# shenyunhang/APE

Hardware: AMD Instinct MI355X
Metric: images/sec @1024^2 APE-L_D fwd (higher is better)
Workload: dtype bf16

## Files before the change

ape_amd/csrc/select.hip:

```cpp
#include "common.h"
#include "../../include/ape_hip.h"

__device__ __forceinline__ bool iou_gt(const float4 a, const float4 b, float thr) {
  const float area_a = (a.z - a.x) * (a.w - a.y);
  const float area_b = (b.z - b.x) * (b.w - b.y);
  const float xx1 = fmaxf(a.x, b.x), yy1 = fmaxf(a.y, b.y);
  const float xx2 = fminf(a.z, b.z), yy2 = fminf(a.w, b.w);
  const float w = fmaxf(0.f, xx2 - xx1), h = fmaxf(0.f, yy2 - yy1);
  const float inter = w * h;
  return inter / (area_a + area_b - inter) > thr;
}

__global__ __launch_bounds__(64) void nms_mask_kernel(const float4* __restrict__ boxes, const int* __restrict__ groups, int n,
                                                      float thr, unsigned long long* __restrict__ mask, int nw) {
  __shared__ float4 cb[64];
  __shared__ int cg[64];
  const int rb = blockIdx.y, cbk = blockIdx.x, t = threadIdx.x;
  const int j0 = cbk * 64;
  if (j0 + t < n) {
    cb[t] = boxes[j0 + t];
    cg[t] = groups ? groups[j0 + t] : 0;
  }
  __syncthreads();
  const int i = rb * 64 + t;
  if (i >= n) return;
  const float4 bi = boxes[i];
  const int gi = groups ? groups[i] : 0;
  unsigned long long bits = 0ull;
  const int cnt = min(64, n - j0);
  for (int j = 0; j < cnt; ++j) {
    if (j0 + j != i && cg[j] == gi && iou_gt(bi, cb[j], thr)) bits |= (1ull << j);
  }
  mask[(size_t)i * nw + cbk] = bits;
}

__device__ __forceinline__ unsigned long long readlane64(unsigned long long v, int lane_uniform) {
  const unsigned lo = (unsigned)__builtin_amdgcn_readlane((int)(unsigned)(v & 0xffffffffull), lane_uniform);
  const unsigned hi = (unsigned)__builtin_amdgcn_readlane((int)(unsigned)(v >> 32), lane_uniform);
  return ((unsigned long long)hi << 32) | lo;
}

__device__ __forceinline__ unsigned long long uniform64(unsigned long long v) {
  const unsigned lo = (unsigned)__builtin_amdgcn_readfirstlane((int)(unsigned)(v & 0xffffffffull));
  const unsigned hi = (unsigned)__builtin_amdgcn_readfirstlane((int)(unsigned)(v >> 32));
  return ((unsigned long long)hi << 32) | lo;
}
__device__ __forceinline__ unsigned long long wave_or64(unsigned long long v) {
  unsigned lo = (unsigned)(v & 0xffffffffull), hi = (unsigned)(v >> 32);
#pragma unroll
  for (int o = 32; o > 0; o >>= 1) { lo |= (unsigned)__shfl_xor((int)lo, o, 64); hi |= (unsigned)__shfl_xor((int)hi, o, 64); }
  return ((unsigned long long)hi << 32) | lo;
}

template <bool USE_LDS>
__global__ __launch_bounds__(256) void nms_scan_segments_kernel(const unsigned long long* __restrict__ mask, int nw, int n,
                                                                const int* __restrict__ seg, const uint8_t* __restrict__ valid,
                                                                uint8_t* __restrict__ keep) {
  extern __shared__ __attribute__((aligned(16))) unsigned long long sub[];
  const int s0 = seg[blockIdx.x], s1 = seg[blockIdx.x + 1];
  if (s1 <= s0) return;
  const int w0 = s0 >> 6, w1 = (s1 - 1) >> 6;
  const int nws = w1 - w0 + 1;
  const int r_base = w0 * 64;
  if (USE_LDS) {
    const int nrows = (w1 + 1) * 64 - r_base;
    for (int e = threadIdx.x; e < nrows * nws; e += 256) {
      const int r = e / nws, w = e - r * nws;
      const int row = r_base + r;
      sub[e] = row < n ? mask[(size_t)row * nw + w0 + w] : 0ull;
    }
    __syncthreads();
  }
  if (threadIdx.x >= 64) return;
  const int lane = threadIdx.x;
  auto word = [&](int row, int c) -> unsigned long long {
    if (USE_LDS) return sub[(size_t)(row - r_base) * nws + (c - w0)];
    return mask[(size_t)(row < n ? row : n - 1) * nw + c];
  };
  unsigned long long kept0 = 0ull, kept1 = 0ull;
  for (int c = w0; c <= w1; ++c) {
    unsigned long long acc = 0ull;
    for (int cp = w0; cp < c; cp += 8) {
      unsigned long long t[8];
#pragma unroll
      for (int u = 0; u < 8; ++u) {
        const int cq = cp + u;
        const int cqc = cq < c ? cq : cp;
        const int rel = cqc - w0;
        const unsigned long long km = readlane64(rel >= 64 ? kept1 : kept0, rel & 63);
        const bool take = cq < c && ((km >> lane) & 1ull);
        const unsigned long long v = word(cqc * 64 + lane, c);
        t[u] = take ? v : 0ull;
      }
#pragma unroll
      for (int u = 0; u < 8; ++u) acc |= t[u];
    }
    const unsigned long long remc = uniform64(wave_or64(acc));
    const int i = c * 64 + lane;
    const bool in_seg = i >= s0 && i < s1;
    const bool ok = in_seg && (valid == nullptr || valid[i] != 0);
    const unsigned long long row_c = ok ? word(i, c) : 0ull;
    unsigned long long alive = __builtin_amdgcn_ballot_w64(ok) & ~remc;
    unsigned long long kept = 0ull;
    while (alive != 0ull) {
      const int j = __builtin_ctzll(alive);
      kept |= 1ull << j;
      alive &= ~(1ull << j);
      alive &= ~readlane64(row_c, j);
    }
    if (in_seg) keep[i] = (uint8_t)((kept >> lane) & 1ull);
    const int rel = c - w0;
    if (lane == (rel & 63)) { if (rel >= 64) kept1 = kept; else kept0 = kept; }
  }
}

__global__ __launch_bounds__(256) void nms_scan_classes_kernel(const unsigned long long* __restrict__ mask, int nw, int n,
                                                               const int* __restrict__ order, const uint8_t* __restrict__ valid,
                                                               uint8_t* __restrict__ keep, int num_classes) {
  extern __shared__ __attribute__((aligned(16))) unsigned long long smask[];
  const int tid = threadIdx.x, lane = tid & 63, wave = tid >> 6;
  for (int i = tid; i < n * nw; i += 256) smask[i] = mask[i];
  __syncthreads();
  const int c = blockIdx.x * 4 + wave;
  if (c >= num_classes) return;
  const int* ord = order + (size_t)c * n;
  unsigned long long rem = 0ull;
  for (int base = 0; base < n; base += 64) {
    const int p = base + lane;
    const int qv = p < n ? ord[p] : 0;
    const int okv = (p < n) && (valid == nullptr || valid[(size_t)c * n + p] != 0);
    int keptv = 0;
    const int cnt = min(64, n - base);
    for (int u = 0; u < cnt; ++u) {
      const int qi = __builtin_amdgcn_readlane(qv, u);
      const int ok = __builtin_amdgcn_readlane(okv, u);
      const unsigned long long row = lane < nw ? smask[(size_t)qi * nw + lane] : 0ull;
      const unsigned long long r = readlane64(rem, qi >> 6);
      const bool kept = ok && !((r >> (qi & 63)) & 1ull);
      if (kept) rem |= row;
      if (lane == u) keptv = kept ? 1 : 0;
    }
    if (p < n) keep[(size_t)c * n + p] = (uint8_t)keptv;
  }
}

extern "C" int ape_hip_nms_mask_words(int n) { return ceil_div(n, 64); }

extern "C" int ape_hip_nms_mask(const float* boxes, const int* groups, int n, float iou_thr, uint64_t* mask, void* stream) {
  APE_CHECK_ARG(boxes && mask && n > 0 && ((uintptr_t)boxes) % 16 == 0, "ape_hip_nms_mask: bad args");
  const int nw = ceil_div(n, 64);
  APE_LAUNCH(nms_mask_kernel, dim3(nw, nw), dim3(64), 0, (hipStream_t)stream, (const float4*)boxes, groups, n, iou_thr,
                     (unsigned long long*)mask, nw);
  APE_CHECK_LAUNCH("ape_hip_nms_mask");
  return 0;
}

extern "C" int ape_hip_nms_scan_segments(const uint64_t* mask, int n, const int* seg_offsets, int num_segments, int max_segment,
                                         const uint8_t* valid, uint8_t* keep, void* stream) {
  APE_CHECK_ARG(mask && seg_offsets && keep && n > 0 && num_segments > 0, "ape_hip_nms_scan_segments: bad args");
  APE_CHECK_ARG(max_segment <= 126 * 64, "ape_hip_nms_scan_segments: segment longer than %d candidates", 126 * 64);
  const size_t sub_rows = (size_t)(ceil_div(max_segment, 64) + 1) * 64, sub_words = (size_t)ceil_div(max_segment, 64) + 1;
  const size_t lds = sub_rows * sub_words * 8;
  if (lds <= 160 * 1024) {
    static ApeOncePerDevice attr_done;
    if (attr_done.first()) {
      (void)hipFuncSetAttribute((const void*)nms_scan_segments_kernel<true>, hipFuncAttributeMaxDynamicSharedMemorySize, 160 * 1024);
    }
    APE_LAUNCH(nms_scan_segments_kernel<true>, dim3(num_segments), dim3(256), lds, (hipStream_t)stream,
                       (const unsigned long long*)mask, ceil_div(n, 64), n, seg_offsets, valid, keep);
  } else {
    APE_LAUNCH(nms_scan_segments_kernel<false>, dim3(num_segments), dim3(256), 0, (hipStream_t)stream,
                       (const unsigned long long*)mask, ceil_div(n, 64), n, seg_offsets, valid, keep);
  }
  APE_CHECK_LAUNCH("ape_hip_nms_scan_segments");
  return 0;
}

extern "C" int ape_hip_nms_scan_classes(const uint64_t* mask, int n, const int* order, int num_classes, const uint8_t* valid,
                                        uint8_t* keep, void* stream) {
  const int nw = ceil_div(n, 64);
  const size_t lds = (size_t)n * nw * 8;
  APE_CHECK_ARG(mask && order && keep && n > 0 && num_classes > 0 && lds <= 160 * 1024,
                "ape_hip_nms_scan_classes: bad args (the n x n/64 bit matrix must fit the 160 KiB LDS: n <= 1280)");
  static ApeOncePerDevice attr_done;
  if (attr_done.first()) {
    (void)hipFuncSetAttribute((const void*)nms_scan_classes_kernel, hipFuncAttributeMaxDynamicSharedMemorySize, 160 * 1024);
  }
  APE_LAUNCH(nms_scan_classes_kernel, dim3(ceil_div(num_classes, 4)), dim3(256), lds, (hipStream_t)stream,
                     (const unsigned long long*)mask, nw, n, order, valid, keep, num_classes);
  APE_CHECK_LAUNCH("ape_hip_nms_scan_classes");
  return 0;
}
```

ape_amd/csrc/topk.hip:

```cpp
#include "common.h"
#include "../../include/ape_hip.h"

typedef unsigned long long u64;
#define TK_THREADS 1024

__device__ __forceinline__ uint32_t ordkey(float x) {
  const uint32_t u = __float_as_uint(x);
  return u ^ ((u >> 31) ? 0xffffffffu : 0x80000000u);
}
__device__ __forceinline__ float ordkey_inv(uint32_t k) {
  return __uint_as_float(k ^ ((k >> 31) ? 0x80000000u : 0xffffffffu));
}
__device__ __forceinline__ float sigmoid_f(float x) { return 1.f / (1.f + expf(-x)); }

struct TkLevels {
  int start[8];
  int n[8];
  int L;
};
__device__ __forceinline__ int level_of(const TkLevels& lv, int idx) {
  int l = 0;
#pragma unroll
  for (int i = 1; i < 8; ++i) l += (i < lv.L && idx >= lv.start[i]) ? 1 : 0;
  return l;
}

template <int N>
__device__ __forceinline__ void bitonic_desc(u64* s) {
  for (int k = 2; k <= N; k <<= 1) {
    for (int j = k >> 1; j > 0; j >>= 1) {
      for (int i = threadIdx.x; i < N; i += TK_THREADS) {
        const int p = i ^ j;
        if (p > i) {
          const u64 a = s[i], b = s[p];
          const bool first_larger = (i & k) == 0;
          if (first_larger ? (a < b) : (a > b)) { s[i] = b; s[p] = a; }
        }
      }
      __syncthreads();
    }
  }
}

template <typename KeyFn>
__device__ __forceinline__ void radix_select(KeyFn key, int n, int k, uint32_t* hist, uint32_t* sh, uint32_t& thr, uint32_t& rem) {
  uint32_t prefix = 0, r = (uint32_t)k;
  for (int shift = 24; shift >= 0; shift -= 8) {
    for (int b = threadIdx.x; b < 256; b += TK_THREADS) hist[b] = 0;
    __syncthreads();
    const uint32_t himask = shift == 24 ? 0u : (0xffffffffu << (shift + 8));
    for (int i0 = 0; i0 < n; i0 += TK_THREADS) {
      const int i = i0 + threadIdx.x;
      const uint32_t kk = i < n ? key(i) : 0u;
      bool live = i < n && (kk & himask) == prefix;
      const uint32_t bin = (kk >> shift) & 255u;
      u64 todo = __ballot(live);
      while (todo) {
        const int leader = __ffsll((long long)todo) - 1;
        const uint32_t lb = (uint32_t)__builtin_amdgcn_readlane((int)bin, leader);
        const u64 same = __ballot(live && bin == lb);
        if ((int)(threadIdx.x & 63) == leader) atomicAdd(&hist[lb], (uint32_t)__popcll(same));
        todo &= ~same;
        if (live && bin == lb) live = false;
      }
    }
    __syncthreads();
    if (threadIdx.x == 0) {
      uint32_t cum = 0;
      int b = 255;
      for (; b > 0; --b) {
        if (cum + hist[b] >= r) break;
        cum += hist[b];
      }
      sh[0] = prefix | ((uint32_t)b << shift);
      sh[1] = r - cum;
    }
    __syncthreads();
    prefix = sh[0];
    r = sh[1];
    __syncthreads();
  }
  thr = prefix;
  rem = r;
}

template <typename KeyFn, typename CompFn>
__device__ __forceinline__ void block_topk(KeyFn key, CompFn composite, int n, int k, u64* comp, uint32_t* hist, uint32_t* sh, uint32_t* wcnt) {
  comp[threadIdx.x] = 0ull;
  __syncthreads();
  if (n <= k) {
    for (int i = threadIdx.x; i < n; i += TK_THREADS) comp[i] = composite(i);
    __syncthreads();
  } else {
    uint32_t thr, rem;
    radix_select(key, n, k, hist, sh, thr, rem);
    const uint32_t ngt = (uint32_t)k - rem;
    const int lane = threadIdx.x & 63, wave = threadIdx.x >> 6;
    uint32_t base_gt = 0, base_eq = 0;
    for (int i0 = 0; i0 < n; i0 += TK_THREADS) {
      const int i = i0 + threadIdx.x;
      const uint32_t kk = i < n ? key(i) : 0u;
      const bool gt = i < n && kk > thr, eq = i < n && kk == thr;
      const u64 bg = __ballot(gt), be = __ballot(eq);
      const u64 lt = (1ull << lane) - 1ull;
      if (lane == 0) { wcnt[wave] = (uint32_t)__popcll(bg); wcnt[16 + wave] = (uint32_t)__popcll(be); }
      __syncthreads();
      uint32_t wg = 0, we = 0, tg = 0, te = 0;
#pragma unroll
      for (int w = 0; w < 16; ++w) {
        const uint32_t cg = wcnt[w], ce = wcnt[16 + w];
        if (w < wave) { wg += cg; we += ce; }
        tg += cg; te += ce;
      }
      if (gt) comp[base_gt + wg + (uint32_t)__popcll(bg & lt)] = composite(i);
      if (eq) {
        const uint32_t rank = base_eq + we + (uint32_t)__popcll(be & lt);
        if (rank < rem) comp[ngt + rank] = composite(i);
      }
      base_gt += tg;
      base_eq += te;
      __syncthreads();
    }
  }
  bitonic_desc<1024>(comp);
}

template <int PER>
__device__ __forceinline__ void block_topk_regs(const uint32_t (&kk)[PER], int n, int k, uint32_t gbase, u64* comp, uint32_t* hist,
                                                uint32_t* sh, uint32_t* wcnt) {
  comp[threadIdx.x] = 0ull;
  __syncthreads();
  const int lane = threadIdx.x & 63, wave = threadIdx.x >> 6;
  if (n <= k) {
    if ((int)threadIdx.x < n) comp[threadIdx.x] = ((u64)kk[0] << 32) | (u64)(0xffffffffu - (gbase + threadIdx.x));
    __syncthreads();
  } else {
    uint32_t prefix = 0, r = (uint32_t)k;
    for (int shift = 24; shift >= 0; shift -= 8) {
      for (int b = threadIdx.x; b < 256; b += TK_THREADS) hist[b] = 0;
      __syncthreads();
      const uint32_t himask = shift == 24 ? 0u : (0xffffffffu << (shift + 8));
#pragma unroll
      for (int j = 0; j < PER; ++j) {
        const int e = j * TK_THREADS + threadIdx.x;
        bool live = e < n && (kk[j] & himask) == prefix;
        const uint32_t bin = (kk[j] >> shift) & 255u;
        u64 todo = __ballot(live);
        while (todo) {
          const int leader = __ffsll((long long)todo) - 1;
          const uint32_t lb = (uint32_t)__builtin_amdgcn_readlane((int)bin, leader);
          const u64 same = __ballot(live && bin == lb);
          if (lane == leader) atomicAdd(&hist[lb], (uint32_t)__popcll(same));
          todo &= ~same;
          if (live && bin == lb) live = false;
        }
      }
      __syncthreads();
      if (threadIdx.x == 0) {
        uint32_t cum = 0;
        int b = 255;
        for (; b > 0; --b) {
          if (cum + hist[b] >= r) break;
          cum += hist[b];
        }
        sh[0] = prefix | ((uint32_t)b << shift);
        sh[1] = r - cum;
      }
      __syncthreads();
      prefix = sh[0];
      r = sh[1];
      __syncthreads();
    }
    const uint32_t thr = prefix, rem = r, ngt = (uint32_t)k - rem;
    uint32_t base_gt = 0, base_eq = 0;
#pragma unroll
    for (int j = 0; j < PER; ++j) {
      const int e = j * TK_THREADS + threadIdx.x;
      const bool gt = e < n && kk[j] > thr, eq = e < n && kk[j] == thr;
      const u64 bg = __ballot(gt), be = __ballot(eq);
      const u64 lt = (1ull << lane) - 1ull;
      if (lane == 0) { wcnt[wave] = (uint32_t)__popcll(bg); wcnt[16 + wave] = (uint32_t)__popcll(be); }
      __syncthreads();
      uint32_t wg = 0, we = 0, tg = 0, te = 0;
#pragma unroll
      for (int w = 0; w < 16; ++w) {
        const uint32_t cg = wcnt[w], ce = wcnt[16 + w];
        if (w < wave) { wg += cg; we += ce; }
        tg += cg; te += ce;
      }
      const u64 c = ((u64)kk[j] << 32) | (u64)(0xffffffffu - (gbase + (uint32_t)e));
      if (gt) comp[base_gt + wg + (uint32_t)__popcll(bg & lt)] = c;
      if (eq) {
        const uint32_t rank = base_eq + we + (uint32_t)__popcll(be & lt);
        if (rank < rem) comp[ngt + rank] = c;
      }
      base_gt += tg;
      base_eq += te;
      __syncthreads();
    }
  }
  bitonic_desc<1024>(comp);
}

#define TK_STAGE2_MAX 12288
#define TK_MAX_JOBS 96
struct TkJobs {
  int njobs, nseg;
  int seg_first[8], seg_jobs[8], seg_k[8], seg_n[8], seg_mode[8];
  int start[TK_MAX_JOBS], n[TK_MAX_JOBS], seg[TK_MAX_JOBS];
};

__device__ __forceinline__ void stage2_gather(const u64* __restrict__ ws, int first_job, int njobs, int k, u64* lds) {
  const int m = njobs * k;
  for (int i = threadIdx.x; i < m; i += TK_THREADS) lds[i] = ws[(size_t)(first_job + i / k) * 1024 + (i % k)];
  __syncthreads();
}

__global__ __launch_bounds__(256) void enc_finalize_kernel(const float* __restrict__ cls2, const float* __restrict__ d,
                                                           const float* __restrict__ anchors, int T, float* __restrict__ enc_class,
                                                           float* __restrict__ enc_coord, float* __restrict__ xyxy) {
  const int t = blockIdx.x * 256 + threadIdx.x;
  if (t >= T) return;
  const float2 c = *reinterpret_cast<const float2*>(cls2 + 2 * (size_t)t);
  const bool pick = c.y > c.x;
  enc_class[t] = pick ? c.y : c.x;
  const float4 dd = *reinterpret_cast<const float4*>(d + 8 * (size_t)t + (pick ? 4 : 0));
  const float4 a = *reinterpret_cast<const float4*>(anchors + 4 * (size_t)t);
  const float4 u = make_float4(dd.x + a.x, dd.y + a.y, dd.z + a.z, dd.w + a.w);
  *reinterpret_cast<float4*>(enc_coord + 4 * (size_t)t) = u;
  const float cx = sigmoid_f(u.x), cy = sigmoid_f(u.y), w = sigmoid_f(u.z), h = sigmoid_f(u.w);
  float4 b = make_float4(cx - 0.5f * w, cy - 0.5f * h, cx + 0.5f * w, cy + 0.5f * h);
  b.x = fminf(fmaxf(b.x, 0.f), 1.f); b.y = fminf(fmaxf(b.y, 0.f), 1.f);
  b.z = fminf(fmaxf(b.z, 0.f), 1.f); b.w = fminf(fmaxf(b.w, 0.f), 1.f);
  *reinterpret_cast<float4*>(xyxy + 4 * (size_t)t) = b;
}

template <int PER>
__global__ __launch_bounds__(TK_THREADS) void topk_stage1_kernel(const float* __restrict__ x, TkJobs jobs, u64* __restrict__ ws) {
  __shared__ u64 comp[1024];
  __shared__ uint32_t hist[256], sh[2], wcnt[32];
  const int job = blockIdx.x, seg = jobs.seg[job], start = jobs.start[job], n = jobs.n[job];
  const bool sig = jobs.seg_mode[seg] != 0;
  uint32_t kk[PER];
#pragma unroll
  for (int j = 0; j < PER; ++j) {
    const int e = j * TK_THREADS + threadIdx.x;
    const float v = e < n ? x[start + e] : 0.f;
    kk[j] = e < n ? ordkey(sig ? sigmoid_f(v) : v + 0.f) : 0u;
  }
  block_topk_regs<PER>(kk, n, jobs.seg_k[seg], (uint32_t)start, comp, hist, sh, wcnt);
  ws[(size_t)job * 1024 + threadIdx.x] = comp[threadIdx.x];
}

__global__ __launch_bounds__(TK_THREADS) void proposal_topk2_kernel(const u64* __restrict__ ws, TkJobs jobs, TkLevels lv, int k, int k_alt,
                                                                    int32_t* __restrict__ cand, int32_t* __restrict__ alt) {
  extern __shared__ u64 lds[];
  __shared__ u64 comp[1024];
  __shared__ uint32_t hist[256], sh[2], wcnt[32];
  const int l = blockIdx.x;
  const int kk = jobs.seg_k[l], m = jobs.seg_jobs[l] * kk;
  stage2_gather(ws, jobs.seg_first[l], jobs.seg_jobs[l], kk, lds);
  auto key = [&](int i) { return (uint32_t)(lds[i] >> 32); };
  auto composite = [&](int i) { return lds[i]; };
  block_topk(key, composite, m, kk, comp, hist, sh, wcnt);
  if (l == lv.L) {
    for (int r = threadIdx.x; r < k_alt; r += TK_THREADS) alt[r] = (int32_t)(0xffffffffu - (uint32_t)(comp[r] & 0xffffffffull));
    return;
  }
  const int start = lv.start[l], n = lv.n[l];
  const int own = n < k ? n : k;
  for (int r = threadIdx.x; r < k; r += TK_THREADS) {
    int idx;
    if (r < own) {
      idx = (int)(0xffffffffu - (uint32_t)(comp[r] & 0xffffffffull));
    } else {
      const int e = r - n;
      idx = e >= start ? e + n : e;
    }
    cand[l * k + r] = idx;
  }
}

__device__ __forceinline__ void scan5(const uint32_t v[5], uint32_t out[5], uint32_t tot[5], u64* sa, uint32_t* sb) {
  const int lane = threadIdx.x & 63, wave = threadIdx.x >> 6;
  u64 a = (u64)v[0] | ((u64)v[1] << 16) | ((u64)v[2] << 32) | ((u64)v[3] << 48);
  uint32_t b = v[4];
  u64 ia = a;
  uint32_t ib = b;
#pragma unroll
  for (int o = 1; o < 64; o <<= 1) {
    const uint32_t lo = __shfl_up((uint32_t)(ia & 0xffffffffull), o, 64), hi = __shfl_up((uint32_t)(ia >> 32), o, 64);
    const uint32_t tb = __shfl_up(ib, o, 64);
    if (lane >= o) { ia += ((u64)hi << 32) | lo; ib += tb; }
  }
  __syncthreads();
  if (lane == 63) { sa[wave] = ia; sb[wave] = ib; }
  __syncthreads();
  u64 wa = 0, ta = 0;
  uint32_t wb = 0, tb2 = 0;
#pragma unroll
  for (int w = 0; w < 16; ++w) {
    if (w < wave) { wa += sa[w]; wb += sb[w]; }
    ta += sa[w]; tb2 += sb[w];
  }
  const u64 ea = wa + ia - a;
  out[0] = (uint32_t)(ea & 0xffff); out[1] = (uint32_t)((ea >> 16) & 0xffff); out[2] = (uint32_t)((ea >> 32) & 0xffff);
  out[3] = (uint32_t)((ea >> 48) & 0xffff); out[4] = wb + ib - b;
  tot[0] = (uint32_t)(ta & 0xffff); tot[1] = (uint32_t)((ta >> 16) & 0xffff); tot[2] = (uint32_t)((ta >> 32) & 0xffff);
  tot[3] = (uint32_t)((ta >> 48) & 0xffff); tot[4] = tb2;
}

#define PO_PAD 8192
#define PO_PER (PO_PAD / TK_THREADS)
__global__ __launch_bounds__(TK_THREADS) void proposal_order_kernel(const int32_t* __restrict__ cand, int n, const float* __restrict__ logit,
                                                                    const float* __restrict__ xyxy, TkLevels lv,
                                                                    float* __restrict__ boxes_b, int32_t* __restrict__ groups_b,
                                                                    int32_t* __restrict__ seg, int32_t* __restrict__ cand_a,
                                                                    int32_t* __restrict__ lv_a, int32_t* __restrict__ pos_b) {
  extern __shared__ u64 po_lds[];
  __shared__ u64 sa[16];
  __shared__ uint32_t sb[16];
  const int nchunks = (n + 1023) >> 10, npad = nchunks << 10;
  u64* work = po_lds;
  u64* srt = po_lds + npad;
  for (int p = threadIdx.x; p < npad; p += TK_THREADS)
    work[p] = p < n ? (((u64)ordkey(logit[cand[p]] + 0.f) << 32) | (u64)(0xffffffffu - (uint32_t)p)) : (u64)(npad - 1 - p);
  __syncthreads();
  for (int k = 2; k <= 1024; k <<= 1) {
    for (int j = k >> 1; j > 0; j >>= 1) {
      for (int i = threadIdx.x; i < npad; i += TK_THREADS) {
        const int q = i ^ j;
        if (q > i) {
          const u64 a = work[i], b = work[q];
          const bool first_larger = ((i & 1023) & k) == 0;
          if (first_larger ? (a < b) : (a > b)) { work[i] = b; work[q] = a; }
        }
      }
      __syncthreads();
    }
  }
  for (int i = threadIdx.x; i < npad; i += TK_THREADS) {
    const u64 v = work[i];
    const int c = i >> 10;
    int rank = i & 1023;
    for (int o = 0; o < nchunks; ++o) {
      if (o == c) continue;
      const u64* ch = work + (o << 10);
      int lo = 0, hi = 1024;
      while (lo < hi) {
        const int mid = (lo + hi) >> 1;
        if (ch[mid] > v) lo = mid + 1; else hi = mid;
      }
      rank += lo;
    }
    srt[rank] = v;
  }
  __syncthreads();
  int idx[PO_PER], lev[PO_PER];
  uint32_t cnt[5] = {0, 0, 0, 0, 0};
#pragma unroll
  for (int j = 0; j < PO_PER; ++j) {
    const int a = threadIdx.x * PO_PER + j;
    idx[j] = -1; lev[j] = 0;
    if (a < n) {
      const int p = (int)(0xffffffffu - (uint32_t)(srt[a] & 0xffffffffull));
      idx[j] = cand[p];
      lev[j] = level_of(lv, idx[j]);
      cnt[lev[j]] += 1;
    }
  }
  uint32_t ex[5], tot[5];
  scan5(cnt, ex, tot, sa, sb);
  uint32_t segs[6];
  segs[0] = 0;
#pragma unroll
  for (int l = 0; l < 5; ++l) segs[l + 1] = segs[l] + tot[l];
  if (threadIdx.x == 0)
    for (int l = 0; l <= lv.L; ++l) seg[l] = (int32_t)segs[l];
#pragma unroll
  for (int j = 0; j < PO_PER; ++j) {
    const int a = threadIdx.x * PO_PER + j;
    if (a < n) {
      const int l = lev[j];
      const int b = (int)(segs[l] + ex[l]);
      ex[l] += 1;
      cand_a[a] = idx[j]; lv_a[a] = l; pos_b[a] = b;
      groups_b[b] = l;
      *reinterpret_cast<float4*>(boxes_b + 4 * (size_t)b) = *reinterpret_cast<const float4*>(xyxy + 4 * (size_t)idx[j]);
    }
  }
}

__global__ __launch_bounds__(TK_THREADS) void proposal_quota_kernel(const int32_t* __restrict__ cand_a, const int32_t* __restrict__ lv_a,
                                                                    const int32_t* __restrict__ pos_b, const uint8_t* __restrict__ keep_b,
                                                                    int n, const int32_t* __restrict__ alt, int n_alt, TkLevels lv, int nq,
                                                                    long long* __restrict__ out) {
  __shared__ u64 sa[16];
  __shared__ uint32_t sb[16];
  int X[PO_PER], lev[PO_PER];
  bool valid[PO_PER];
  uint32_t c[5] = {0, 0, 0, 0, 0};
#pragma unroll
  for (int j = 0; j < PO_PER; ++j) {
    const int a = threadIdx.x * PO_PER + j;
    X[j] = 0; lev[j] = 0; valid[j] = false;
    if (a < n) {
      X[j] = cand_a[a]; lev[j] = lv_a[a];
      valid[j] = keep_b[pos_b[a]] != 0;
      c[0] += valid[j] ? 1u : 0u;
    }
  }
  uint32_t ex[5], tot[5];
  scan5(c, ex, tot, sa, sb);
  const bool use_alt = (int)tot[0] < nq;
  if (use_alt) {
#pragma unroll
    for (int j = 0; j < PO_PER; ++j) {
      const int a = threadIdx.x * PO_PER + j;
      valid[j] = a < n && a < n_alt;
      X[j] = valid[j] ? alt[a] : 0;
      lev[j] = level_of(lv, X[j]);
    }
  }
  for (int r = threadIdx.x; r < nq; r += TK_THREADS) out[r] = 0;
#pragma unroll
  for (int l = 0; l < 5; ++l) c[l] = 0;
#pragma unroll
  for (int j = 0; j < PO_PER; ++j)
    if (valid[j]) c[lev[j]] += 1;
  scan5(c, ex, tot, sa, sb);
  const uint32_t quota = (uint32_t)(nq / lv.L);
  bool sel[PO_PER];
  uint32_t c2[5] = {0, 0, 0, 0, 0};
#pragma unroll
  for (int j = 0; j < PO_PER; ++j) {
    sel[j] = false;
    if (valid[j]) {
      sel[j] = ex[lev[j]] < quota;
      ex[lev[j]] += 1;
      c2[sel[j] ? 0 : 1] += 1;
    }
  }
  scan5(c2, ex, tot, sa, sb);
  const uint32_t need = (uint32_t)nq - tot[0];
  uint32_t c3[5] = {0, 0, 0, 0, 0};
  uint32_t rest = ex[1];
#pragma unroll
  for (int j = 0; j < PO_PER; ++j) {
    if (valid[j] && !sel[j]) {
      if (rest < need) sel[j] = true;
      rest += 1;
    }
    c3[0] += sel[j] ? 1u : 0u;
  }
  scan5(c3, ex, tot, sa, sb);
  uint32_t slot = ex[0];
#pragma unroll
  for (int j = 0; j < PO_PER; ++j)
    if (sel[j]) {
      if (slot < (uint32_t)nq) out[slot] = (long long)X[j];
      slot += 1;
    }
}

__global__ __launch_bounds__(64) void det_boxes_kernel(const float* __restrict__ logits, int ldl, int K, const float* __restrict__ boxes,
                                                       const float* __restrict__ scale, float* __restrict__ xyxy,
                                                       uint8_t* __restrict__ finite) {
  const int q = blockIdx.x, lane = threadIdx.x;
  bool ok = true;
  for (int c = lane; c < K; c += 64) ok = ok && isfinite(sigmoid_f(logits[(size_t)q * ldl + c]));
  ok = __ballot(!ok) == 0ull;
  if (lane == 0) {
    const float4 b = *reinterpret_cast<const float4*>(boxes + 4 * (size_t)q);
    const float4 s = *reinterpret_cast<const float4*>(scale);
    float4 o = make_float4((b.x - 0.5f * b.z) * s.x, (b.y - 0.5f * b.w) * s.y, (b.x + 0.5f * b.z) * s.z, (b.y + 0.5f * b.w) * s.w);
    ok = ok && isfinite(o.x) && isfinite(o.y) && isfinite(o.z) && isfinite(o.w);
    o.x = fminf(fmaxf(o.x, 0.f), s.x); o.y = fminf(fmaxf(o.y, 0.f), s.y);
    o.z = fminf(fmaxf(o.z, 0.f), s.z); o.w = fminf(fmaxf(o.w, 0.f), s.w);
    if (!ok) o = make_float4(0.f, 0.f, 0.f, 0.f);
    *reinterpret_cast<float4*>(xyxy + 4 * (size_t)q) = o;
    finite[q] = ok ? 1 : 0;
  }
}

__global__ __launch_bounds__(TK_THREADS) void class_sort_kernel(const float* __restrict__ logits, int ldl, int Q, const uint8_t* __restrict__ finite,
                                                                float thresh, float* __restrict__ sorted, int32_t* __restrict__ order,
                                                                uint8_t* __restrict__ valid) {
  __shared__ u64 comp[1024];
  const int c = blockIdx.x, q = threadIdx.x;
  comp[q] = q < Q ? (((u64)ordkey(sigmoid_f(logits[(size_t)q * ldl + c])) << 32) | (u64)(0xffffffffu - (uint32_t)q)) : 0ull;
  __syncthreads();
  bitonic_desc<1024>(comp);
  if (q < Q) {
    const float s = ordkey_inv((uint32_t)(comp[q] >> 32));
    const int src = (int)(0xffffffffu - (uint32_t)(comp[q] & 0xffffffffull));
    sorted[(size_t)c * Q + q] = s;
    order[(size_t)c * Q + q] = src;
    valid[(size_t)c * Q + q] = (s > thresh && finite[src]) ? 1 : 0;
  }
}

template <int PER>
__global__ __launch_bounds__(TK_THREADS) void det_topk1_kernel(const float* __restrict__ sorted, const uint8_t* __restrict__ keep, int total,
                                                               int k, u64* __restrict__ ws) {
  __shared__ u64 comp[1024];
  __shared__ uint32_t hist[256], sh[2], wcnt[32];
  const int start = blockIdx.x * (PER * TK_THREADS);
  const int n = min(PER * TK_THREADS, total - start);
  uint32_t kk[PER];
#pragma unroll
  for (int j = 0; j < PER; ++j) {
    const int e = j * TK_THREADS + threadIdx.x;
    kk[j] = e < n ? ordkey(keep[start + e] ? sorted[start + e] : -1.f) : 0u;
  }
  block_topk_regs<PER>(kk, n, k, (uint32_t)start, comp, hist, sh, wcnt);
  ws[(size_t)blockIdx.x * 1024 + threadIdx.x] = comp[threadIdx.x];
}

__global__ __launch_bounds__(TK_THREADS) void topk_merge_kernel(const u64* __restrict__ in, int nlists, int group, int k, u64* __restrict__ out) {
  extern __shared__ u64 lds[];
  __shared__ u64 comp[1024];
  __shared__ uint32_t hist[256], sh[2], wcnt[32];
  const int first = blockIdx.x * group;
  const int cnt = min(group, nlists - first);
  stage2_gather(in, first, cnt, k, lds);
  auto key = [&](int i) { return (uint32_t)(lds[i] >> 32); };
  auto composite = [&](int i) { return lds[i]; };
  block_topk(key, composite, cnt * k, k, comp, hist, sh, wcnt);
  out[(size_t)blockIdx.x * 1024 + threadIdx.x] = comp[threadIdx.x];
}

__global__ __launch_bounds__(TK_THREADS) void det_topk2_kernel(const u64* __restrict__ ws, int nchunks, const int32_t* __restrict__ order,
                                                               const float* __restrict__ xyxy, int Q, int k, float* __restrict__ det_boxes,
                                                               float* __restrict__ det_scores, long long* __restrict__ det_classes,
                                                               long long* __restrict__ det_query) {
  extern __shared__ u64 lds[];
  __shared__ u64 comp[1024];
  __shared__ uint32_t hist[256], sh[2], wcnt[32];
  stage2_gather(ws, 0, nchunks, k, lds);
  auto key = [&](int i) { return (uint32_t)(lds[i] >> 32); };
  auto composite = [&](int i) { return lds[i]; };
  block_topk(key, composite, nchunks * k, k, comp, hist, sh, wcnt);
  for (int r = threadIdx.x; r < k; r += TK_THREADS) {
    const int flat = (int)(0xffffffffu - (uint32_t)(comp[r] & 0xffffffffull));
    const int qi = order[flat];
    det_scores[r] = ordkey_inv((uint32_t)(comp[r] >> 32));
    det_classes[r] = (long long)(flat / Q);
    det_query[r] = (long long)qi;
    *reinterpret_cast<float4*>(det_boxes + 4 * (size_t)r) = *reinterpret_cast<const float4*>(xyxy + 4 * (size_t)qi);
  }
}

static int fill_levels(TkLevels& lv, const int* level_start, const int* level_n, int L) {
  APE_CHECK_ARG(level_start && level_n && L >= 1 && L <= 5, "proposal selection: 1 <= levels <= 5");
  for (int i = 0; i < 8; ++i) { lv.start[i] = i < L ? level_start[i] : 0x7fffffff; lv.n[i] = i < L ? level_n[i] : 0; }
  lv.L = L;
  return 0;
}

extern "C" int ape_hip_enc_finalize(const float* cls2, const float* d, const float* anchors, int T, float* enc_class, float* enc_coord,
                                    float* xyxy, void* stream) {
  APE_CHECK_ARG(cls2 && d && anchors && enc_class && enc_coord && xyxy && T > 0, "ape_hip_enc_finalize: bad arguments");
  APE_LAUNCH(enc_finalize_kernel, dim3(ceil_div(T, 256)), dim3(256), 0, (hipStream_t)stream, cls2, d, anchors, T, enc_class,
                     enc_coord, xyxy);
  APE_CHECK_LAUNCH("enc_finalize_kernel");
  return 0;
}

static int topk_per(const int* seg_n, const int* seg_k, int nseg) {
  const int pers[3] = {8, 32, 64};
  for (int pi = 0; pi < 3; ++pi) {
    bool ok = true;
    int jobs = 0;
    for (int s = 0; s < nseg; ++s) {
      const int c = ceil_div(seg_n[s], pers[pi] * TK_THREADS);
      ok = ok && (long long)c * seg_k[s] <= TK_STAGE2_MAX;
      jobs += c;
    }
    if (ok && jobs <= TK_MAX_JOBS) return pers[pi];
  }
  return 0;
}

static void set_stage2_attr() {
  static ApeOncePerDevice done;
  if (done.first()) {
    (void)hipFuncSetAttribute((const void*)proposal_topk2_kernel, hipFuncAttributeMaxDynamicSharedMemorySize, 112 * 1024);
    (void)hipFuncSetAttribute((const void*)det_topk2_kernel, hipFuncAttributeMaxDynamicSharedMemorySize, 112 * 1024);
    (void)hipFuncSetAttribute((const void*)topk_merge_kernel, hipFuncAttributeMaxDynamicSharedMemorySize, 112 * 1024);
  }
}

extern "C" int ape_hip_topk_workspace_words(int n_total) {
  const int det = ceil_div(n_total > 0 ? n_total : 1, 8 * TK_THREADS);
  const int lists = det > TK_MAX_JOBS ? det : TK_MAX_JOBS;
  return 1024 * (lists + lists / 2 + 1);
}

extern "C" int ape_hip_proposal_topk(const float* logit, int T, const int* level_start, const int* level_n, int L, int k, int k_alt,
                                     uint64_t* workspace, int32_t* cand, int32_t* alt, void* stream) {
  TkLevels lv;
  if (fill_levels(lv, level_start, level_n, L)) return -1;
  APE_CHECK_ARG(logit && workspace && cand && alt && T > 0 && k >= 1 && k <= 1024 && k_alt >= 1 && k_alt <= 1024 && k <= T && k_alt <= T,
                "ape_hip_proposal_topk: 1 <= k, k_alt <= min(1024, T)");
  int seg_n[8], seg_k[8];
  for (int l = 0; l < L; ++l) { seg_n[l] = level_n[l]; seg_k[l] = k; }
  seg_n[L] = T; seg_k[L] = k_alt;
  const int per = topk_per(seg_n, seg_k, L + 1);
  APE_CHECK_ARG(per > 0, "ape_hip_proposal_topk: %d tokens do not fit the two-stage selection", T);
  TkJobs jobs;
  memset(&jobs, 0, sizeof(jobs));
  jobs.nseg = L + 1;
  const int chunk = per * TK_THREADS;
  for (int s = 0; s <= L; ++s) {
    const int base = s < L ? level_start[s] : 0;
    jobs.seg_first[s] = jobs.njobs; jobs.seg_k[s] = seg_k[s]; jobs.seg_n[s] = seg_n[s]; jobs.seg_mode[s] = s < L ? 1 : 0;
    for (int c0 = 0; c0 < seg_n[s]; c0 += chunk) {
      jobs.start[jobs.njobs] = base + c0; jobs.n[jobs.njobs] = seg_n[s] - c0 < chunk ? seg_n[s] - c0 : chunk; jobs.seg[jobs.njobs] = s;
      ++jobs.njobs;
    }
    jobs.seg_jobs[s] = jobs.njobs - jobs.seg_first[s];
  }
  hipStream_t st = (hipStream_t)stream;
  u64* ws = reinterpret_cast<u64*>(workspace);
  if (per == 8) APE_LAUNCH(topk_stage1_kernel<8>, dim3(jobs.njobs), dim3(TK_THREADS), 0, st, logit, jobs, ws);
  else if (per == 32) APE_LAUNCH(topk_stage1_kernel<32>, dim3(jobs.njobs), dim3(TK_THREADS), 0, st, logit, jobs, ws);
  else APE_LAUNCH(topk_stage1_kernel<64>, dim3(jobs.njobs), dim3(TK_THREADS), 0, st, logit, jobs, ws);
  set_stage2_attr();
  int mmax = 0;
  for (int s = 0; s <= L; ++s) mmax = mmax > jobs.seg_jobs[s] * jobs.seg_k[s] ? mmax : jobs.seg_jobs[s] * jobs.seg_k[s];
  APE_LAUNCH(proposal_topk2_kernel, dim3(L + 1), dim3(TK_THREADS), (size_t)mmax * sizeof(u64), st, ws, jobs, lv, k, k_alt, cand, alt);
  APE_CHECK_LAUNCH("proposal_topk");
  return 0;
}

extern "C" int ape_hip_proposal_order(const int32_t* cand, int n, const float* logit, const float* xyxy, const int* level_start,
                                      const int* level_n, int L, float* boxes_b, int32_t* groups_b, int32_t* seg, int32_t* cand_a,
                                      int32_t* lv_a, int32_t* pos_b, void* stream) {
  TkLevels lv;
  if (fill_levels(lv, level_start, level_n, L)) return -1;
  APE_CHECK_ARG(cand && logit && xyxy && boxes_b && groups_b && seg && cand_a && lv_a && pos_b && n > 0 && n <= PO_PAD,
                "ape_hip_proposal_order: 1 <= n <= 8192 candidates");
  static ApeOncePerDevice attr_done;
  if (attr_done.first()) {
    (void)hipFuncSetAttribute((const void*)proposal_order_kernel, hipFuncAttributeMaxDynamicSharedMemorySize, 2 * PO_PAD * sizeof(u64));
  }
  APE_LAUNCH(proposal_order_kernel, dim3(1), dim3(TK_THREADS), (size_t)2 * ((n + 1023) / 1024) * 1024 * sizeof(u64), (hipStream_t)stream, cand, n, logit, xyxy, lv,
                     boxes_b, groups_b, seg, cand_a, lv_a, pos_b);
  APE_CHECK_LAUNCH("proposal_order_kernel");
  return 0;
}

extern "C" int ape_hip_proposal_quota(const int32_t* cand_a, const int32_t* lv_a, const int32_t* pos_b, const uint8_t* keep_b, int n,
                                      const int32_t* alt, int n_alt, const int* level_start, const int* level_n, int L, int nq,
                                      int64_t* out, void* stream) {
  TkLevels lv;
  if (fill_levels(lv, level_start, level_n, L)) return -1;
  APE_CHECK_ARG(cand_a && lv_a && pos_b && keep_b && alt && out && n > 0 && n <= PO_PAD && n_alt >= 0 && nq > 0,
                "ape_hip_proposal_quota: bad arguments (n <= 8192)");
  APE_LAUNCH(proposal_quota_kernel, dim3(1), dim3(TK_THREADS), 0, (hipStream_t)stream, cand_a, lv_a, pos_b, keep_b, n, alt, n_alt,
                     lv, nq, (long long*)out);
  APE_CHECK_LAUNCH("proposal_quota_kernel");
  return 0;
}

extern "C" int ape_hip_det_sort(const float* logits, int ldl, int Q, int K, const float* boxes, const float* scale, float thresh,
                                float* xyxy, uint8_t* finite, float* sorted, int32_t* order, uint8_t* valid, void* stream) {
  APE_CHECK_ARG(logits && boxes && scale && xyxy && finite && sorted && order && valid && K > 0, "ape_hip_det_sort: bad arguments");
  APE_CHECK_ARG(Q > 0 && Q <= 1024, "ape_hip_det_sort: 1 <= queries <= 1024 (got %d)", Q);
  hipStream_t st = (hipStream_t)stream;
  APE_LAUNCH(det_boxes_kernel, dim3(Q), dim3(64), 0, st, logits, ldl, K, boxes, scale, xyxy, finite);
  APE_LAUNCH(class_sort_kernel, dim3(K), dim3(TK_THREADS), 0, st, logits, ldl, Q, finite, thresh, sorted, order, valid);
  APE_CHECK_LAUNCH("ape_hip_det_sort");
  return 0;
}

extern "C" int ape_hip_det_topk(const float* sorted, const uint8_t* keep, const int32_t* order, const float* xyxy, int K, int Q, int k,
                                uint64_t* workspace, float* det_boxes, float* det_scores, int64_t* det_classes, int64_t* det_query,
                                void* stream) {
  APE_CHECK_ARG(sorted && keep && order && xyxy && workspace && det_boxes && det_scores && det_classes && det_query, "ape_hip_det_topk: null pointer");
  APE_CHECK_ARG(K > 0 && Q > 0 && (long long)K * Q < 0x7fffffffLL && k >= 1 && k <= 1024 && k <= K * Q, "ape_hip_det_topk: 1 <= k <= min(1024, K*Q)");
  const int total = K * Q;
  int per = topk_per(&total, &k, 1);
  const bool merge = per == 0;
  if (merge) per = 64;
  int nchunks = ceil_div(total, per * TK_THREADS);
  hipStream_t st = (hipStream_t)stream;
  u64* ws = reinterpret_cast<u64*>(workspace);
  if (per == 8) APE_LAUNCH(det_topk1_kernel<8>, dim3(nchunks), dim3(TK_THREADS), 0, st, sorted, keep, total, k, ws);
  else if (per == 32) APE_LAUNCH(det_topk1_kernel<32>, dim3(nchunks), dim3(TK_THREADS), 0, st, sorted, keep, total, k, ws);
  else APE_LAUNCH(det_topk1_kernel<64>, dim3(nchunks), dim3(TK_THREADS), 0, st, sorted, keep, total, k, ws);
  set_stage2_attr();
  if (merge) {
    const int cap_lists = ape_hip_topk_workspace_words(total) / 1024;
    u64* a = ws;
    u64* b = ws + (size_t)1024 * (cap_lists - (cap_lists / 3));
    const int group = TK_STAGE2_MAX / k;
    while ((long long)nchunks * k > TK_STAGE2_MAX) {
      const int nout = ceil_div(nchunks, group);
      APE_LAUNCH(topk_merge_kernel, dim3(nout), dim3(TK_THREADS), (size_t)group * k * sizeof(u64), st, a, nchunks, group, k, b);
      u64* t = a; a = b; b = t;
      nchunks = nout;
    }
    ws = a;
  }
  APE_LAUNCH(det_topk2_kernel, dim3(1), dim3(TK_THREADS), (size_t)nchunks * k * sizeof(u64), st, ws, nchunks, order, xyxy, Q, k,
                     det_boxes, det_scores, (long long*)det_classes, (long long*)det_query);
  APE_CHECK_LAUNCH("det_topk");
  return 0;
}
```

Baseline: 117.9.

## Rework NMS scans and top-k selection with register sorts and staged LDS

The segment NMS scan now stages mask columns into LDS in column groups, double-buffered, so three waves prefetch the next group while one wave scans. This replaces the old fallback that read from global memory whenever the segment did not fit. The per-class NMS scan now skips suppressed candidates in bulk via ballots instead of walking every candidate serially, and gains a global-memory fallback. Top-k and class sorting replace LDS bitonic sorts with register and lane-shuffle bitonic networks, and the stage-2 selection no longer gathers into dynamic LDS. These post-processing kernels are a small share of the end-to-end forward pass, and the large rewrite carries correctness risk.

Result: no change. 118.6, median of 6 (+0.6%).

```diff
diff --git a/ape_amd/csrc/select.hip b/ape_amd/csrc/select.hip
--- a/ape_amd/csrc/select.hip
+++ b/ape_amd/csrc/select.hip
@@ -52,95 +52,131 @@
   return ((unsigned long long)hi << 32) | lo;
 }
 
-template <bool USE_LDS>
+__device__ __forceinline__ void nms_stage_columns(const unsigned long long* __restrict__ mask, int nw, int n, int r_base, int c_first, int ncols,
+                                                  int nrows, int rows_cap, unsigned long long* buf, int tid, int nthreads) {
+  const int total = nrows * ncols;
+  for (int e0 = tid; e0 < total; e0 += 8 * nthreads) {
+    unsigned long long v[8];
+#pragma unroll
+    for (int u = 0; u < 8; ++u) {
+      const int e = min(e0 + u * nthreads, total - 1);
+      const int r = e / ncols, w = e - r * ncols;
+      v[u] = mask[(size_t)min(r_base + r, n - 1) * nw + c_first + w];
+    }
+#pragma unroll
+    for (int u = 0; u < 8; ++u) {
+      const int e = e0 + u * nthreads;
+      const int r = e / ncols, w = e - r * ncols;
+      if (e < total) buf[(size_t)w * rows_cap + r] = r_base + r < n ? v[u] : 0ull;
+    }
+  }
+}
+
 __global__ __launch_bounds__(256) void nms_scan_segments_kernel(const unsigned long long* __restrict__ mask, int nw, int n,
                                                                 const int* __restrict__ seg, const uint8_t* __restrict__ valid,
-                                                                uint8_t* __restrict__ keep) {
+                                                                uint8_t* __restrict__ keep, int gcols, int rows_cap) {
   extern __shared__ __attribute__((aligned(16))) unsigned long long sub[];
   const int s0 = seg[blockIdx.x], s1 = seg[blockIdx.x + 1];
   if (s1 <= s0) return;
   const int w0 = s0 >> 6, w1 = (s1 - 1) >> 6;
-  const int nws = w1 - w0 + 1;
   const int r_base = w0 * 64;
-  if (USE_LDS) {
-    const int nrows = (w1 + 1) * 64 - r_base;
-    for (int e = threadIdx.x; e < nrows * nws; e += 256) {
-      const int r = e / nws, w = e - r * nws;
-      const int row = r_base + r;
-      sub[e] = row < n ? mask[(size_t)row * nw + w0 + w] : 0ull;
+  if ((w1 - w0 + 1) * 64 > rows_cap) return;
+  const int lane = threadIdx.x & 63, wave = threadIdx.x >> 6;
+  const int ngroups = (w1 - w0 + gcols) / gcols;
+  auto group_cols = [&](int g) { return min(gcols, w1 + 1 - (w0 + g * gcols)); };
+  auto group_rows = [&](int g) { return (g * gcols + group_cols(g)) * 64; };
+  nms_stage_columns(mask, nw, n, r_base, w0, group_cols(0), group_rows(0), rows_cap, sub, threadIdx.x, 256);
+  __syncthreads();
+  unsigned long long kept0 = 0ull, kept1 = 0ull;
+  for (int g = 0; g < ngroups; ++g) {
+    const unsigned long long* cur = sub + (size_t)(g & 1) * gcols * rows_cap;
+    const int c_lo = w0 + g * gcols, c_hi = c_lo + group_cols(g) - 1;
+    if (wave != 0) {
+      if (g + 1 < ngroups)
+        nms_stage_columns(mask, nw, n, r_base, c_lo + gcols, group_cols(g + 1), group_rows(g + 1), rows_cap,
+                          sub + (size_t)((g + 1) & 1) * gcols * rows_cap, threadIdx.x - 64, 192);
+    } else {
+      auto word = [&](int row, int c) -> unsigned long long {
+        return cur[(size_t)(c - c_lo) * rows_cap + (row - r_base)];
+      };
+      for (int c = c_lo; c <= c_hi; ++c) {
+        unsigned long long acc = 0ull;
+        for (int cp = w0; cp < c; cp += 8) {
+          unsigned long long t[8];
+#pragma unroll
+          for (int u = 0; u < 8; ++u) {
+            const int cq = cp + u;
+            const int cqc = cq < c ? cq : cp;
+            const int rel = cqc - w0;
+            const unsigned long long km = readlane64(rel >= 64 ? kept1 : kept0, rel & 63);
+            const bool take = cq < c && ((km >> lane) & 1ull);
+            const unsigned long long v = word(cqc * 64 + lane, c);
+            t[u] = take ? v : 0ull;
+          }
+#pragma unroll
+          for (int u = 0; u < 8; ++u) acc |= t[u];
+        }
+        const unsigned long long remc = uniform64(wave_or64(acc));
+        const int i = c * 64 + lane;
+        const bool in_seg = i >= s0 && i < s1;
+        const bool ok = in_seg && (valid == nullptr || valid[i] != 0);
+        const unsigned long long row_c = ok ? word(i, c) : 0ull;
+        unsigned long long alive = __builtin_amdgcn_ballot_w64(ok) & ~remc;
+        unsigned long long kept = 0ull;
+        while (alive != 0ull) {
+          const int j = __builtin_ctzll(alive);
+          kept |= 1ull << j;
+          alive &= ~(1ull << j);
+          alive &= ~readlane64(row_c, j);
+        }
+        if (in_seg) keep[i] = (uint8_t)((kept >> lane) & 1ull);
+        const int rel = c - w0;
+        if (lane == (rel & 63)) { if (rel >= 64) kept1 = kept; else kept0 = kept; }
+      }
     }
     __syncthreads();
   }
-  if (threadIdx.x >= 64) return;
-  const int lane = threadIdx.x;
-  auto word = [&](int row, int c) -> unsigned long long {
-    if (USE_LDS) return sub[(size_t)(row - r_base) * nws + (c - w0)];
-    return mask[(size_t)(row < n ? row : n - 1) * nw + c];
-  };
-  unsigned long long kept0 = 0ull, kept1 = 0ull;
-  for (int c = w0; c <= w1; ++c) {
-    unsigned long long acc = 0ull;
-    for (int cp = w0; cp < c; cp += 8) {
-      unsigned long long t[8];
-#pragma unroll
-      for (int u = 0; u < 8; ++u) {
-        const int cq = cp + u;
-        const int cqc = cq < c ? cq : cp;
-        const int rel = cqc - w0;
-        const unsigned long long km = readlane64(rel >= 64 ? kept1 : kept0, rel & 63);
-        const bool take = cq < c && ((km >> lane) & 1ull);
-        const unsigned long long v = word(cqc * 64 + lane, c);
-        t[u] = take ? v : 0ull;
-      }
-#pragma unroll
-      for (int u = 0; u < 8; ++u) acc |= t[u];
-    }
-    const unsigned long long remc = uniform64(wave_or64(acc));
-    const int i = c * 64 + lane;
-    const bool in_seg = i >= s0 && i < s1;
-    const bool ok = in_seg && (valid == nullptr || valid[i] != 0);
-    const unsigned long long row_c = ok ? word(i, c) : 0ull;
-    unsigned long long alive = __builtin_amdgcn_ballot_w64(ok) & ~remc;
+}
+
+template <bool IN_LDS>
+__global__ __launch_bounds__(256) void nms_scan_classes_kernel(const unsigned long long* __restrict__ mask, int nw, int n,
+                                                               const int* __restrict__ order, const uint8_t* __restrict__ valid,
+                                                               uint8_t* __restrict__ keep, int num_classes) {
+  extern __shared__ __attribute__((aligned(16))) unsigned long long lds_mask[];
+  const int tid = threadIdx.x, lane = tid & 63, wave = tid >> 6;
+  if (IN_LDS) {
+    for (int i = tid; i < n * nw; i += 256) lds_mask[i] = mask[i];
+    __syncthreads();
+  }
+  const unsigned long long* smask = IN_LDS ? lds_mask : mask;
+  const int c = blockIdx.x * 4 + wave;
+  if (c >= num_classes) return;
+  const int* ord = order + (size_t)c * n;
+  const uint8_t* val = valid ? valid + (size_t)c * n : nullptr;
+  unsigned long long rem = 0ull;
+  int qv = lane < n ? ord[lane] : 0;
+  bool okv = lane < n && (val == nullptr || val[lane] != 0);
+  for (int base = 0; base < n; base += 64) {
+    const int p = base + lane, pn = p + 64;
+    const int q_next = pn < n ? ord[pn] : 0;
+    const bool ok_next = pn < n && (val == nullptr || val[pn] != 0);
+    const int qw = qv >> 6, qb = qv & 63;
+    const unsigned lo = (unsigned)__shfl((int)(unsigned)(rem & 0xffffffffull), qw, 64), hi = (unsigned)__shfl((int)(unsigned)(rem >> 32), qw, 64);
+    const unsigned long long own = ((unsigned long long)hi << 32) | lo;
+    unsigned long long alive = __builtin_amdgcn_ballot_w64(okv && !((own >> qb) & 1ull));
     unsigned long long kept = 0ull;
     while (alive != 0ull) {
       const int j = __builtin_ctzll(alive);
       kept |= 1ull << j;
+      const unsigned long long* row = smask + (size_t)__builtin_amdgcn_readlane(qv, j) * nw;
+      if (lane < nw) rem |= row[lane];
+      const unsigned long long hit = __builtin_amdgcn_ballot_w64((row[qw] >> qb) & 1ull);
       alive &= ~(1ull << j);
-      alive &= ~readlane64(row_c, j);
-    }
-    if (in_seg) keep[i] = (uint8_t)((kept >> lane) & 1ull);
-    const int rel = c - w0;
-    if (lane == (rel & 63)) { if (rel >= 64) kept1 = kept; else kept0 = kept; }
-  }
-}
-
-__global__ __launch_bounds__(256) void nms_scan_classes_kernel(const unsigned long long* __restrict__ mask, int nw, int n,
-                                                               const int* __restrict__ order, const uint8_t* __restrict__ valid,
-                                                               uint8_t* __restrict__ keep, int num_classes) {
-  extern __shared__ __attribute__((aligned(16))) unsigned long long smask[];
-  const int tid = threadIdx.x, lane = tid & 63, wave = tid >> 6;
-  for (int i = tid; i < n * nw; i += 256) smask[i] = mask[i];
-  __syncthreads();
-  const int c = blockIdx.x * 4 + wave;
-  if (c >= num_classes) return;
-  const int* ord = order + (size_t)c * n;
-  unsigned long long rem = 0ull;
-  for (int base = 0; base < n; base += 64) {
-    const int p = base + lane;
-    const int qv = p < n ? ord[p] : 0;
-    const int okv = (p < n) && (valid == nullptr || valid[(size_t)c * n + p] != 0);
-    int keptv = 0;
-    const int cnt = min(64, n - base);
-    for (int u = 0; u < cnt; ++u) {
-      const int qi = __builtin_amdgcn_readlane(qv, u);
-      const int ok = __builtin_amdgcn_readlane(okv, u);
-      const unsigned long long row = lane < nw ? smask[(size_t)qi * nw + lane] : 0ull;
-      const unsigned long long r = readlane64(rem, qi >> 6);
-      const bool kept = ok && !((r >> (qi & 63)) & 1ull);
-      if (kept) rem |= row;
-      if (lane == u) keptv = kept ? 1 : 0;
-    }
-    if (p < n) keep[(size_t)c * n + p] = (uint8_t)keptv;
+      alive &= ~hit;
+    }
+    if (p < n) keep[(size_t)c * n + p] = (uint8_t)((kept >> lane) & 1ull);
+    qv = q_next;
+    okv = ok_next;
   }
 }
 
@@ -159,19 +195,20 @@
                                          const uint8_t* valid, uint8_t* keep, void* stream) {
   APE_CHECK_ARG(mask && seg_offsets && keep && n > 0 && num_segments > 0, "ape_hip_nms_scan_segments: bad args");
   APE_CHECK_ARG(max_segment <= 126 * 64, "ape_hip_nms_scan_segments: segment longer than %d candidates", 126 * 64);
-  const size_t sub_rows = (size_t)(ceil_div(max_segment, 64) + 1) * 64, sub_words = (size_t)ceil_div(max_segment, 64) + 1;
-  const size_t lds = sub_rows * sub_words * 8;
-  if (lds <= 160 * 1024) {
-    static ApeOncePerDevice attr_done;
-    if (attr_done.first()) {
-      (void)hipFuncSetAttribute((const void*)nms_scan_segments_kernel<true>, hipFuncAttributeMaxDynamicSharedMemorySize, 160 * 1024);
-    }
-    APE_LAUNCH(nms_scan_segments_kernel<true>, dim3(num_segments), dim3(256), lds, (hipStream_t)stream,
-                       (const unsigned long long*)mask, ceil_div(n, 64), n, seg_offsets, valid, keep);
-  } else {
-    APE_LAUNCH(nms_scan_segments_kernel<false>, dim3(num_segments), dim3(256), 0, (hipStream_t)stream,
-                       (const unsigned long long*)mask, ceil_div(n, 64), n, seg_offsets, valid, keep);
-  }
+  const int max_chunks = ceil_div(max_segment > 0 ? max_segment : 1, 64) + 1, rows_cap = max_chunks * 64;
+  const size_t col_bytes = (size_t)rows_cap * 8, lds_max = 160 * 1024;
+  int gcols = max_chunks;
+  size_t lds = col_bytes * gcols;
+  if (lds > lds_max) {
+    gcols = (int)(lds_max / 2 / col_bytes);
+    lds = 2 * col_bytes * gcols;
+  }
+  static ApeOncePerDevice attr_done;
+  if (attr_done.first()) {
+    (void)hipFuncSetAttribute((const void*)nms_scan_segments_kernel, hipFuncAttributeMaxDynamicSharedMemorySize, 160 * 1024);
+  }
+  APE_LAUNCH(nms_scan_segments_kernel, dim3(num_segments), dim3(256), lds, (hipStream_t)stream,
+                     (const unsigned long long*)mask, ceil_div(n, 64), n, seg_offsets, valid, keep, gcols, rows_cap);
   APE_CHECK_LAUNCH("ape_hip_nms_scan_segments");
   return 0;
 }
@@ -180,14 +217,19 @@
                                         uint8_t* keep, void* stream) {
   const int nw = ceil_div(n, 64);
   const size_t lds = (size_t)n * nw * 8;
-  APE_CHECK_ARG(mask && order && keep && n > 0 && num_classes > 0 && lds <= 160 * 1024,
+  APE_CHECK_ARG(mask && order && keep && n > 0 && num_classes > 0 && n <= 1280,
                 "ape_hip_nms_scan_classes: bad args (the n x n/64 bit matrix must fit the 160 KiB LDS: n <= 1280)");
-  static ApeOncePerDevice attr_done;
-  if (attr_done.first()) {
-    (void)hipFuncSetAttribute((const void*)nms_scan_classes_kernel, hipFuncAttributeMaxDynamicSharedMemorySize, 160 * 1024);
-  }
-  APE_LAUNCH(nms_scan_classes_kernel, dim3(ceil_div(num_classes, 4)), dim3(256), lds, (hipStream_t)stream,
-                     (const unsigned long long*)mask, nw, n, order, valid, keep, num_classes);
+  if (lds <= 160 * 1024) {
+    static ApeOncePerDevice attr_done;
+    if (attr_done.first()) {
+      (void)hipFuncSetAttribute((const void*)nms_scan_classes_kernel<true>, hipFuncAttributeMaxDynamicSharedMemorySize, 160 * 1024);
+    }
+    APE_LAUNCH(nms_scan_classes_kernel<true>, dim3(ceil_div(num_classes, 4)), dim3(256), lds, (hipStream_t)stream,
+                       (const unsigned long long*)mask, nw, n, order, valid, keep, num_classes);
+  } else {
+    APE_LAUNCH(nms_scan_classes_kernel<false>, dim3(ceil_div(num_classes, 4)), dim3(256), 0, (hipStream_t)stream,
+                       (const unsigned long long*)mask, nw, n, order, valid, keep, num_classes);
+  }
   APE_CHECK_LAUNCH("ape_hip_nms_scan_classes");
   return 0;
 }
diff --git a/ape_amd/csrc/topk.hip b/ape_amd/csrc/topk.hip
--- a/ape_amd/csrc/topk.hip
+++ b/ape_amd/csrc/topk.hip
@@ -25,184 +25,172 @@
   return l;
 }
 
-template <int N>
-__device__ __forceinline__ void bitonic_desc(u64* s) {
+__device__ __forceinline__ u64 lane_xor64(u64 v, int j) {
+  const uint32_t lo = __shfl_xor((uint32_t)(v & 0xffffffffull), j, 64), hi = __shfl_xor((uint32_t)(v >> 32), j, 64);
+  return ((u64)hi << 32) | lo;
+}
+__device__ __forceinline__ int pow2_at_least(int n) {
+  int p = 64;
+  while (p < n) p <<= 1;
+  return p;
+}
+
+template <int NS>
+__device__ __forceinline__ void sort_desc(u64 (&v)[NS], int nseq, int N, u64* xa, u64* xb) {
+  const int t = threadIdx.x;
+  bool second = false;
   for (int k = 2; k <= N; k <<= 1) {
+    const bool desc = k == N || (t & k) == 0;
     for (int j = k >> 1; j > 0; j >>= 1) {
-      for (int i = threadIdx.x; i < N; i += TK_THREADS) {
-        const int p = i ^ j;
-        if (p > i) {
-          const u64 a = s[i], b = s[p];
-          const bool first_larger = (i & k) == 0;
-          if (first_larger ? (a < b) : (a > b)) { s[i] = b; s[p] = a; }
+      const u64* x = nullptr;
+      if (j >= 64) {
+        u64* w = second ? xb : xa;
+        second = !second;
+#pragma unroll
+        for (int c = 0; c < NS; ++c)
+          if (c < nseq) w[c * 1024 + t] = v[c];
+        __syncthreads();
+        x = w;
+      }
+      const bool keep_larger = ((t & j) == 0) == desc;
+#pragma unroll
+      for (int c = 0; c < NS; ++c)
+        if (c < nseq) {
+          const u64 o = j >= 64 ? x[c * 1024 + (t ^ j)] : lane_xor64(v[c], j);
+          v[c] = keep_larger ? (v[c] > o ? v[c] : o) : (v[c] < o ? v[c] : o);
         }
-      }
-      __syncthreads();
-    }
-  }
-}
-
-template <typename KeyFn>
-__device__ __forceinline__ void radix_select(KeyFn key, int n, int k, uint32_t* hist, uint32_t* sh, uint32_t& thr, uint32_t& rem) {
+    }
+  }
+}
+__device__ __forceinline__ u64 sort_desc1(u64 v, int N, u64* xa, u64* xb) {
+  u64 a[1] = {v};
+  sort_desc<1>(a, 1, N, xa, xb);
+  return a[0];
+}
+
+#define TK_SELECT_LDS(PER)                                                  \
+  __shared__ u64 comp[1024];                                                \
+  __shared__ u64 xbuf[1024];                                                \
+  __shared__ __attribute__((aligned(16))) uint32_t hist[256];               \
+  __shared__ __attribute__((aligned(16))) uint32_t wcnt[(PER) * 32];        \
+  __shared__ uint32_t sh[2]
+
+__device__ __forceinline__ void radix_threshold(const uint32_t* hist, uint32_t prefix, uint32_t r, int shift, uint32_t* sh) {
+  const int lane = threadIdx.x & 63;
+  const uint4 h = reinterpret_cast<const uint4*>(hist)[lane];
+  const uint32_t own = h.x + h.y + h.z + h.w;
+  uint32_t suf = own;
+#pragma unroll
+  for (int o = 1; o < 64; o <<= 1) {
+    const uint32_t up = __shfl_down(suf, o, 64);
+    if (lane + o < 64) suf += up;
+  }
+  const u64 reach = __ballot(suf >= r);
+  const int L = reach ? 63 - __builtin_clzll(reach) : 0;
+  if (lane == L) {
+    uint32_t cum = suf - own;
+    int b = 4 * lane + 3;
+    if (cum + h.w < r) { cum += h.w; --b;
+      if (cum + h.z < r) { cum += h.z; --b;
+        if (cum + h.y < r) { cum += h.y; --b; } } }
+    sh[0] = prefix | ((uint32_t)b << shift);
+    sh[1] = r - cum;
+  }
+}
+
+template <int PER, typename KeyFn, typename CompFn>
+__device__ __forceinline__ void block_select(KeyFn key, CompFn composite, int n, int k, u64* comp, uint32_t* hist, uint32_t* sh, uint32_t* wcnt) {
+  const int lane = threadIdx.x & 63, wave = threadIdx.x >> 6;
+  const int nslots = (n + TK_THREADS - 1) / TK_THREADS;
+  comp[threadIdx.x] = 0ull;
+  if (n <= k) {
+    if ((int)threadIdx.x < n) comp[threadIdx.x] = composite(0);
+    __syncthreads();
+    return;
+  }
   uint32_t prefix = 0, r = (uint32_t)k;
   for (int shift = 24; shift >= 0; shift -= 8) {
-    for (int b = threadIdx.x; b < 256; b += TK_THREADS) hist[b] = 0;
+    if (threadIdx.x < 256) hist[threadIdx.x] = 0;
     __syncthreads();
     const uint32_t himask = shift == 24 ? 0u : (0xffffffffu << (shift + 8));
-    for (int i0 = 0; i0 < n; i0 += TK_THREADS) {
-      const int i = i0 + threadIdx.x;
-      const uint32_t kk = i < n ? key(i) : 0u;
-      bool live = i < n && (kk & himask) == prefix;
-      const uint32_t bin = (kk >> shift) & 255u;
-      u64 todo = __ballot(live);
-      while (todo) {
-        const int leader = __ffsll((long long)todo) - 1;
-        const uint32_t lb = (uint32_t)__builtin_amdgcn_readlane((int)bin, leader);
-        const u64 same = __ballot(live && bin == lb);
-        if ((int)(threadIdx.x & 63) == leader) atomicAdd(&hist[lb], (uint32_t)__popcll(same));
-        todo &= ~same;
-        if (live && bin == lb) live = false;
-      }
-    }
-    __syncthreads();
-    if (threadIdx.x == 0) {
-      uint32_t cum = 0;
-      int b = 255;
-      for (; b > 0; --b) {
-        if (cum + hist[b] >= r) break;
-        cum += hist[b];
-      }
-      sh[0] = prefix | ((uint32_t)b << shift);
-      sh[1] = r - cum;
-    }
-    __syncthreads();
-    prefix = sh[0];
-    r = sh[1];
-    __syncthreads();
-  }
-  thr = prefix;
-  rem = r;
-}
-
-template <typename KeyFn, typename CompFn>
-__device__ __forceinline__ void block_topk(KeyFn key, CompFn composite, int n, int k, u64* comp, uint32_t* hist, uint32_t* sh, uint32_t* wcnt) {
-  comp[threadIdx.x] = 0ull;
-  __syncthreads();
-  if (n <= k) {
-    for (int i = threadIdx.x; i < n; i += TK_THREADS) comp[i] = composite(i);
-    __syncthreads();
-  } else {
-    uint32_t thr, rem;
-    radix_select(key, n, k, hist, sh, thr, rem);
-    const uint32_t ngt = (uint32_t)k - rem;
-    const int lane = threadIdx.x & 63, wave = threadIdx.x >> 6;
-    uint32_t base_gt = 0, base_eq = 0;
-    for (int i0 = 0; i0 < n; i0 += TK_THREADS) {
-      const int i = i0 + threadIdx.x;
-      const uint32_t kk = i < n ? key(i) : 0u;
-      const bool gt = i < n && kk > thr, eq = i < n && kk == thr;
-      const u64 bg = __ballot(gt), be = __ballot(eq);
-      const u64 lt = (1ull << lane) - 1ull;
-      if (lane == 0) { wcnt[wave] = (uint32_t)__popcll(bg); wcnt[16 + wave] = (uint32_t)__popcll(be); }
-      __syncthreads();
-      uint32_t wg = 0, we = 0, tg = 0, te = 0;
-#pragma unroll
-      for (int w = 0; w < 16; ++w) {
-        const uint32_t cg = wcnt[w], ce = wcnt[16 + w];
-        if (w < wave) { wg += cg; we += ce; }
-        tg += cg; te += ce;
-      }
-      if (gt) comp[base_gt + wg + (uint32_t)__popcll(bg & lt)] = composite(i);
-      if (eq) {
-        const uint32_t rank = base_eq + we + (uint32_t)__popcll(be & lt);
-        if (rank < rem) comp[ngt + rank] = composite(i);
-      }
-      base_gt += tg;
-      base_eq += te;
-      __syncthreads();
-    }
-  }
-  bitonic_desc<1024>(comp);
-}
-
-template <int PER>
-__device__ __forceinline__ void block_topk_regs(const uint32_t (&kk)[PER], int n, int k, uint32_t gbase, u64* comp, uint32_t* hist,
-                                                uint32_t* sh, uint32_t* wcnt) {
-  comp[threadIdx.x] = 0ull;
-  __syncthreads();
-  const int lane = threadIdx.x & 63, wave = threadIdx.x >> 6;
-  if (n <= k) {
-    if ((int)threadIdx.x < n) comp[threadIdx.x] = ((u64)kk[0] << 32) | (u64)(0xffffffffu - (gbase + threadIdx.x));
-    __syncthreads();
-  } else {
-    uint32_t prefix = 0, r = (uint32_t)k;
-    for (int shift = 24; shift >= 0; shift -= 8) {
-      for (int b = threadIdx.x; b < 256; b += TK_THREADS) hist[b] = 0;
-      __syncthreads();
-      const uint32_t himask = shift == 24 ? 0u : (0xffffffffu << (shift + 8));
-#pragma unroll
-      for (int j = 0; j < PER; ++j) {
+#pragma unroll
+    for (int j = 0; j < PER; ++j) {
+      if (j < nslots) {
         const int e = j * TK_THREADS + threadIdx.x;
-        bool live = e < n && (kk[j] & himask) == prefix;
-        const uint32_t bin = (kk[j] >> shift) & 255u;
+        const uint32_t kj = key(j);
+        bool live = e < n && (kj & himask) == prefix;
+        const uint32_t bin = (kj >> shift) & 255u;
         u64 todo = __ballot(live);
-        while (todo) {
+        if (shift == 24) {
+          while (todo) {
+            const int leader = __ffsll((long long)todo) - 1;
+            const uint32_t lb = (uint32_t)__builtin_amdgcn_readlane((int)bin, leader);
+            const u64 same = __ballot(live && bin == lb);
+            if (lane == leader) atomicAdd(&hist[lb], (uint32_t)__popcll(same));
+            todo &= ~same;
+            if (live && bin == lb) live = false;
+          }
+        } else if (todo) {
           const int leader = __ffsll((long long)todo) - 1;
           const uint32_t lb = (uint32_t)__builtin_amdgcn_readlane((int)bin, leader);
           const u64 same = __ballot(live && bin == lb);
           if (lane == leader) atomicAdd(&hist[lb], (uint32_t)__popcll(same));
-          todo &= ~same;
-          if (live && bin == lb) live = false;
+          else if (live && bin != lb) atomicAdd(&hist[bin], 1u);
         }
       }
-      __syncthreads();
-      if (threadIdx.x == 0) {
-        uint32_t cum = 0;
-        int b = 255;
-        for (; b > 0; --b) {
-          if (cum + hist[b] >= r) break;
-          cum += hist[b];
+    }
+    __syncthreads();
+    if (wave == 0) radix_threshold(hist, prefix, r, shift, sh);
+    __syncthreads();
+    prefix = sh[0];
+    r = sh[1];
+  }
+  const uint32_t thr = prefix, rem = r, ngt = (uint32_t)k - rem;
+  const u64 below = (1ull << lane) - 1ull;
+#pragma unroll
+  for (int j = 0; j < PER; ++j) {
+    if (j < nslots) {
+      const int e = j * TK_THREADS + threadIdx.x;
+      const uint32_t kj = key(j);
+      const u64 bg = __ballot(e < n && kj > thr), be = __ballot(e < n && kj == thr);
+      if (lane == 0) { wcnt[j * 32 + wave] = (uint32_t)__popcll(bg); wcnt[j * 32 + 16 + wave] = (uint32_t)__popcll(be); }
+    }
+  }
+  __syncthreads();
+  uint32_t base_gt = 0, base_eq = 0;
+#pragma unroll
+  for (int j = 0; j < PER; ++j) {
+    if (j < nslots) {
+      const int e = j * TK_THREADS + threadIdx.x;
+      const uint32_t kj = key(j);
+      const bool gt = e < n && kj > thr, eq = e < n && kj == thr;
+      const u64 bg = __ballot(gt), be = __ballot(eq);
+      uint32_t wg = 0, we = 0, tg = 0, te = 0;
+      const uint4* q = reinterpret_cast<const uint4*>(wcnt + j * 32);
+#pragma unroll
+      for (int w4 = 0; w4 < 4; ++w4) {
+        const uint4 cg = q[w4], ce = q[4 + w4];
+        const uint32_t g[4] = {cg.x, cg.y, cg.z, cg.w}, q4[4] = {ce.x, ce.y, ce.z, ce.w};
+#pragma unroll
+        for (int u = 0; u < 4; ++u) {
+          if (w4 * 4 + u < wave) { wg += g[u]; we += q4[u]; }
+          tg += g[u]; te += q4[u];
         }
-        sh[0] = prefix | ((uint32_t)b << shift);
-        sh[1] = r - cum;
       }
-      __syncthreads();
-      prefix = sh[0];
-      r = sh[1];
-      __syncthreads();
-    }
-    const uint32_t thr = prefix, rem = r, ngt = (uint32_t)k - rem;
-    uint32_t base_gt = 0, base_eq = 0;
-#pragma unroll
-    for (int j = 0; j < PER; ++j) {
-      const int e = j * TK_THREADS + threadIdx.x;
-      const bool gt = e < n && kk[j] > thr, eq = e < n && kk[j] == thr;
-      const u64 bg = __ballot(gt), be = __ballot(eq);
-      const u64 lt = (1ull << lane) - 1ull;
-      if (lane == 0) { wcnt[wave] = (uint32_t)__popcll(bg); wcnt[16 + wave] = (uint32_t)__popcll(be); }
-      __syncthreads();
-      uint32_t wg = 0, we = 0, tg = 0, te = 0;
-#pragma unroll
-      for (int w = 0; w < 16; ++w) {
-        const uint32_t cg = wcnt[w], ce = wcnt[16 + w];
-        if (w < wave) { wg += cg; we += ce; }
-        tg += cg; te += ce;
-      }
-      const u64 c = ((u64)kk[j] << 32) | (u64)(0xffffffffu - (gbase + (uint32_t)e));
-      if (gt) comp[base_gt + wg + (uint32_t)__popcll(bg & lt)] = c;
+      if (gt) comp[base_gt + wg + (uint32_t)__popcll(bg & below)] = composite(j);
       if (eq) {
-        const uint32_t rank = base_eq + we + (uint32_t)__popcll(be & lt);
-        if (rank < rem) comp[ngt + rank] = c;
+        const uint32_t rank = base_eq + we + (uint32_t)__popcll(be & below);
+        if (rank < rem) comp[ngt + rank] = composite(j);
       }
       base_gt += tg;
       base_eq += te;
-      __syncthreads();
-    }
-  }
-  bitonic_desc<1024>(comp);
-}
-
-#define TK_STAGE2_MAX 12288
+    }
+  }
+  __syncthreads();
+}
+
+#define TK_STAGE2_PER 12
+#define TK_STAGE2_MAX (TK_STAGE2_PER * 1024)
 #define TK_MAX_JOBS 96
 struct TkJobs {
   int njobs, nseg;
@@ -210,9 +198,23 @@
   int start[TK_MAX_JOBS], n[TK_MAX_JOBS], seg[TK_MAX_JOBS];
 };
 
-__device__ __forceinline__ void stage2_gather(const u64* __restrict__ ws, int first_job, int njobs, int k, u64* lds) {
+__device__ __forceinline__ void stage2_select(const u64* __restrict__ ws, int first_job, int njobs, int k, u64* comp, uint32_t* hist, uint32_t* sh,
+                                              uint32_t* wcnt) {
   const int m = njobs * k;
-  for (int i = threadIdx.x; i < m; i += TK_THREADS) lds[i] = ws[(size_t)(first_job + i / k) * 1024 + (i % k)];
+  u64 c[TK_STAGE2_PER];
+#pragma unroll
+  for (int j = 0; j < TK_STAGE2_PER; ++j) {
+    const int i = j * TK_THREADS + threadIdx.x;
+    c[j] = i < m ? ws[(size_t)(first_job + i / k) * 1024 + (i % k)] : 0ull;
+  }
+  auto key = [&](int j) { return (uint32_t)(c[j] >> 32); };
+  auto composite = [&](int j) { return c[j]; };
+  block_select<TK_STAGE2_PER>(key, composite, m, k, comp, hist, sh, wcnt);
+}
+__device__ __forceinline__ void sort_selected(u64* comp, u64* xbuf, int cnt) {
+  const u64 v = sort_desc1(comp[threadIdx.x], pow2_at_least(cnt), comp, xbuf);
+  __syncthreads();
+  comp[threadIdx.x] = v;
   __syncthreads();
 }
 
@@ -237,9 +239,8 @@
 
 template <int PER>
 __global__ __launch_bounds__(TK_THREADS) void topk_stage1_kernel(const float* __restrict__ x, TkJobs jobs, u64* __restrict__ ws) {
-  __shared__ u64 comp[1024];
-  __shared__ uint32_t hist[256], sh[2], wcnt[32];
-  const int job = blockIdx.x, seg = jobs.seg[job], start = jobs.start[job], n = jobs.n[job];
+  TK_SELECT_LDS(PER);
+  const int job = blockIdx.x, seg = jobs.seg[job], start = jobs.start[job], n = jobs.n[job], k = jobs.seg_k[seg];
   const bool sig = jobs.seg_mode[seg] != 0;
   uint32_t kk[PER];
 #pragma unroll
@@ -248,21 +249,21 @@
     const float v = e < n ? x[start + e] : 0.f;
     kk[j] = e < n ? ordkey(sig ? sigmoid_f(v) : v + 0.f) : 0u;
   }
-  block_topk_regs<PER>(kk, n, jobs.seg_k[seg], (uint32_t)start, comp, hist, sh, wcnt);
-  ws[(size_t)job * 1024 + threadIdx.x] = comp[threadIdx.x];
+  auto key = [&](int j) { return kk[j]; };
+  auto composite = [&](int j) { return ((u64)kk[j] << 32) | (u64)(0xffffffffu - ((uint32_t)start + (uint32_t)(j * TK_THREADS) + threadIdx.x)); };
+  block_select<PER>(key, composite, n, k, comp, hist, sh, wcnt);
+  u64 v = comp[threadIdx.x];
+  if (n <= k) v = sort_desc1(v, pow2_at_least(n), comp, xbuf);
+  ws[(size_t)job * 1024 + threadIdx.x] = v;
 }
 
 __global__ __launch_bounds__(TK_THREADS) void proposal_topk2_kernel(const u64* __restrict__ ws, TkJobs jobs, TkLevels lv, int k, int k_alt,
                                                                     int32_t* __restrict__ cand, int32_t* __restrict__ alt) {
-  extern __shared__ u64 lds[];
-  __shared__ u64 comp[1024];
-  __shared__ uint32_t hist[256], sh[2], wcnt[32];
+  TK_SELECT_LDS(TK_STAGE2_PER);
   const int l = blockIdx.x;
   const int kk = jobs.seg_k[l], m = jobs.seg_jobs[l] * kk;
-  stage2_gather(ws, jobs.seg_first[l], jobs.seg_jobs[l], kk, lds);
-  auto key = [&](int i) { return (uint32_t)(lds[i] >> 32); };
-  auto composite = [&](int i) { return lds[i]; };
-  block_topk(key, composite, m, kk, comp, hist, sh, wcnt);
+  stage2_select(ws, jobs.seg_first[l], jobs.seg_jobs[l], kk, comp, hist, sh, wcnt);
+  sort_selected(comp, xbuf, kk < m ? kk : m);
   if (l == lv.L) {
     for (int r = threadIdx.x; r < k_alt; r += TK_THREADS) alt[r] = (int32_t)(0xffffffffu - (uint32_t)(comp[r] & 0xffffffffull));
     return;
@@ -323,22 +324,18 @@
   const int nchunks = (n + 1023) >> 10, npad = nchunks << 10;
   u64* work = po_lds;
   u64* srt = po_lds + npad;
-  for (int p = threadIdx.x; p < npad; p += TK_THREADS)
-    work[p] = p < n ? (((u64)ordkey(logit[cand[p]] + 0.f) << 32) | (u64)(0xffffffffu - (uint32_t)p)) : (u64)(npad - 1 - p);
-  __syncthreads();
-  for (int k = 2; k <= 1024; k <<= 1) {
-    for (int j = k >> 1; j > 0; j >>= 1) {
-      for (int i = threadIdx.x; i < npad; i += TK_THREADS) {
-        const int q = i ^ j;
-        if (q > i) {
-          const u64 a = work[i], b = work[q];
-          const bool first_larger = ((i & 1023) & k) == 0;
-          if (first_larger ? (a < b) : (a > b)) { work[i] = b; work[q] = a; }
-        }
-      }
-      __syncthreads();
-    }
-  }
+  u64 el[PO_PER];
+#pragma unroll
+  for (int c = 0; c < PO_PER; ++c) {
+    const int p = c * TK_THREADS + threadIdx.x;
+    el[c] = p < n ? (((u64)ordkey(logit[cand[p]] + 0.f) << 32) | (u64)(0xffffffffu - (uint32_t)p)) : (u64)(npad - 1 - p);
+  }
+  sort_desc<PO_PER>(el, nchunks, 1024, work, srt);
+  __syncthreads();
+#pragma unroll
+  for (int c = 0; c < PO_PER; ++c)
+    if (c < nchunks) work[c * TK_THREADS + threadIdx.x] = el[c];
+  __syncthreads();
   for (int i = threadIdx.x; i < npad; i += TK_THREADS) {
     const u64 v = work[i];
     const int c = i >> 10;
@@ -486,14 +483,13 @@
 __global__ __launch_bounds__(TK_THREADS) void class_sort_kernel(const float* __restrict__ logits, int ldl, int Q, const uint8_t* __restrict__ finite,
                                                                 float thresh, float* __restrict__ sorted, int32_t* __restrict__ order,
                                                                 uint8_t* __restrict__ valid) {
-  __shared__ u64 comp[1024];
+  __shared__ u64 xa[1024], xb[1024];
   const int c = blockIdx.x, q = threadIdx.x;
-  comp[q] = q < Q ? (((u64)ordkey(sigmoid_f(logits[(size_t)q * ldl + c])) << 32) | (u64)(0xffffffffu - (uint32_t)q)) : 0ull;
-  __syncthreads();
-  bitonic_desc<1024>(comp);
+  const u64 mine = q < Q ? (((u64)ordkey(sigmoid_f(logits[(size_t)q * ldl + c])) << 32) | (u64)(0xffffffffu - (uint32_t)q)) : 0ull;
+  const u64 v = sort_desc1(mine, pow2_at_least(Q), xa, xb);
   if (q < Q) {
-    const float s = ordkey_inv((uint32_t)(comp[q] >> 32));
-    const int src = (int)(0xffffffffu - (uint32_t)(comp[q] & 0xffffffffull));
+    const float s = ordkey_inv((uint32_t)(v >> 32));
+    const int src = (int)(0xffffffffu - (uint32_t)(v & 0xffffffffull));
     sorted[(size_t)c * Q + q] = s;
     order[(size_t)c * Q + q] = src;
     valid[(size_t)c * Q + q] = (s > thresh && finite[src]) ? 1 : 0;
@@ -503,8 +499,7 @@
 template <int PER>
 __global__ __launch_bounds__(TK_THREADS) void det_topk1_kernel(const float* __restrict__ sorted, const uint8_t* __restrict__ keep, int total,
                                                                int k, u64* __restrict__ ws) {
-  __shared__ u64 comp[1024];
-  __shared__ uint32_t hist[256], sh[2], wcnt[32];
+  TK_SELECT_LDS(PER);
   const int start = blockIdx.x * (PER * TK_THREADS);
   const int n = min(PER * TK_THREADS, total - start);
   uint32_t kk[PER];
@@ -513,20 +508,20 @@
     const int e = j * TK_THREADS + threadIdx.x;
     kk[j] = e < n ? ordkey(keep[start + e] ? sorted[start + e] : -1.f) : 0u;
   }
-  block_topk_regs<PER>(kk, n, k, (uint32_t)start, comp, hist, sh, wcnt);
-  ws[(size_t)blockIdx.x * 1024 + threadIdx.x] = comp[threadIdx.x];
+  auto key = [&](int j) { return kk[j]; };
+  auto composite = [&](int j) { return ((u64)kk[j] << 32) | (u64)(0xffffffffu - ((uint32_t)start + (uint32_t)(j * TK_THREADS) + threadIdx.x)); };
+  block_select<PER>(key, composite, n, k, comp, hist, sh, wcnt);
+  u64 v = comp[threadIdx.x];
+  if (n <= k) v = sort_desc1(v, pow2_at_least(n), comp, xbuf);
+  ws[(size_t)blockIdx.x * 1024 + threadIdx.x] = v;
 }
 
 __global__ __launch_bounds__(TK_THREADS) void topk_merge_kernel(const u64* __restrict__ in, int nlists, int group, int k, u64* __restrict__ out) {
-  extern __shared__ u64 lds[];
-  __shared__ u64 comp[1024];
-  __shared__ uint32_t hist[256], sh[2], wcnt[32];
+  TK_SELECT_LDS(TK_STAGE2_PER);
   const int first = blockIdx.x * group;
   const int cnt = min(group, nlists - first);
-  stage2_gather(in, first, cnt, k, lds);
-  auto key = [&](int i) { return (uint32_t)(lds[i] >> 32); };
-  auto composite = [&](int i) { return lds[i]; };
-  block_topk(key, composite, cnt * k, k, comp, hist, sh, wcnt);
+  stage2_select(in, first, cnt, k, comp, hist, sh, wcnt);
+  (void)xbuf;
   out[(size_t)blockIdx.x * 1024 + threadIdx.x] = comp[threadIdx.x];
 }
 
@@ -534,13 +529,9 @@
                                                                const float* __restrict__ xyxy, int Q, int k, float* __restrict__ det_boxes,
                                                                float* __restrict__ det_scores, long long* __restrict__ det_classes,
                                                                long long* __restrict__ det_query) {
-  extern __shared__ u64 lds[];
-  __shared__ u64 comp[1024];
-  __shared__ uint32_t hist[256], sh[2], wcnt[32];
-  stage2_gather(ws, 0, nchunks, k, lds);
-  auto key = [&](int i) { return (uint32_t)(lds[i] >> 32); };
-  auto composite = [&](int i) { return lds[i]; };
-  block_topk(key, composite, nchunks * k, k, comp, hist, sh, wcnt);
+  TK_SELECT_LDS(TK_STAGE2_PER);
+  stage2_select(ws, 0, nchunks, k, comp, hist, sh, wcnt);
+  sort_selected(comp, xbuf, k);
   for (int r = threadIdx.x; r < k; r += TK_THREADS) {
     const int flat = (int)(0xffffffffu - (uint32_t)(comp[r] & 0xffffffffull));
     const int qi = order[flat];
@@ -580,15 +571,6 @@
     if (ok && jobs <= TK_MAX_JOBS) return pers[pi];
   }
   return 0;
-}
-
-static void set_stage2_attr() {
-  static ApeOncePerDevice done;
-  if (done.first()) {
-    (void)hipFuncSetAttribute((const void*)proposal_topk2_kernel, hipFuncAttributeMaxDynamicSharedMemorySize, 112 * 1024);
-    (void)hipFuncSetAttribute((const void*)det_topk2_kernel, hipFuncAttributeMaxDynamicSharedMemorySize, 112 * 1024);
-    (void)hipFuncSetAttribute((const void*)topk_merge_kernel, hipFuncAttributeMaxDynamicSharedMemorySize, 112 * 1024);
-  }
 }
 
 extern "C" int ape_hip_topk_workspace_words(int n_total) {
@@ -626,10 +608,7 @@
   if (per == 8) APE_LAUNCH(topk_stage1_kernel<8>, dim3(jobs.njobs), dim3(TK_THREADS), 0, st, logit, jobs, ws);
   else if (per == 32) APE_LAUNCH(topk_stage1_kernel<32>, dim3(jobs.njobs), dim3(TK_THREADS), 0, st, logit, jobs, ws);
   else APE_LAUNCH(topk_stage1_kernel<64>, dim3(jobs.njobs), dim3(TK_THREADS), 0, st, logit, jobs, ws);
-  set_stage2_attr();
-  int mmax = 0;
-  for (int s = 0; s <= L; ++s) mmax = mmax > jobs.seg_jobs[s] * jobs.seg_k[s] ? mmax : jobs.seg_jobs[s] * jobs.seg_k[s];
-  APE_LAUNCH(proposal_topk2_kernel, dim3(L + 1), dim3(TK_THREADS), (size_t)mmax * sizeof(u64), st, ws, jobs, lv, k, k_alt, cand, alt);
+  APE_LAUNCH(proposal_topk2_kernel, dim3(L + 1), dim3(TK_THREADS), 0, st, ws, jobs, lv, k, k_alt, cand, alt);
   APE_CHECK_LAUNCH("proposal_topk");
   return 0;
 }
@@ -690,7 +669,6 @@
   if (per == 8) APE_LAUNCH(det_topk1_kernel<8>, dim3(nchunks), dim3(TK_THREADS), 0, st, sorted, keep, total, k, ws);
   else if (per == 32) APE_LAUNCH(det_topk1_kernel<32>, dim3(nchunks), dim3(TK_THREADS), 0, st, sorted, keep, total, k, ws);
   else APE_LAUNCH(det_topk1_kernel<64>, dim3(nchunks), dim3(TK_THREADS), 0, st, sorted, keep, total, k, ws);
-  set_stage2_attr();
   if (merge) {
     const int cap_lists = ape_hip_topk_workspace_words(total) / 1024;
     u64* a = ws;
@@ -698,13 +676,13 @@
     const int group = TK_STAGE2_MAX / k;
     while ((long long)nchunks * k > TK_STAGE2_MAX) {
       const int nout = ceil_div(nchunks, group);
-      APE_LAUNCH(topk_merge_kernel, dim3(nout), dim3(TK_THREADS), (size_t)group * k * sizeof(u64), st, a, nchunks, group, k, b);
+      APE_LAUNCH(topk_merge_kernel, dim3(nout), dim3(TK_THREADS), 0, st, a, nchunks, group, k, b);
       u64* t = a; a = b; b = t;
       nchunks = nout;
     }
     ws = a;
   }
-  APE_LAUNCH(det_topk2_kernel, dim3(1), dim3(TK_THREADS), (size_t)nchunks * k * sizeof(u64), st, ws, nchunks, order, xyxy, Q, k,
+  APE_LAUNCH(det_topk2_kernel, dim3(1), dim3(TK_THREADS), 0, st, ws, nchunks, order, xyxy, Q, k,
                      det_boxes, det_scores, (long long*)det_classes, (long long*)det_query);
   APE_CHECK_LAUNCH("det_topk");
   return 0;
```
